# alibaba/TorchEasyRec

Hardware: AMD Instinct MI355X
Metric: samples/sec DLRM-Criteo (examples/dlrm_criteo.config) training, batch 65536 global (higher is better)
Workload: dtype f32; 1 GPU; dlrm_criteo: 26 tables x dim 16 (204.2M rows, fp32), fused sparse adagrad + dense Adam, ids uniform; global_batch=65536, per_rank_batch=65536, parallelism=single GPU, all tables local (table-wise on one rank), row_layout=interleaved

## Files before the change

include/tzrec_hip.h:

```cpp
#ifndef TZREC_HIP_H_
#define TZREC_HIP_H_

#include <stddef.h>
#include <stdint.h>

#ifdef __cplusplus
extern "C" {
#endif

#define TZR_DT_F32 0
#define TZR_DT_F16 1

#define TZR_OK 0
#define TZR_ERR_INVALID (-1)
#define TZR_ERR_LAUNCH (-2)
#define TZR_ERR_WORKSPACE (-3)
#define TZR_ERR_UNSUPPORTED (-4)

#define TZR_MAX_DST 8
#define TZR_MAX_FEAT_DST 4

#define TZR_POOL_SUM 0
#define TZR_POOL_MEAN 1

// ... 556 lines not shown
                            float* d_grad_sparse, int64_t grad_sparse_stride, void* stream);

int tzr_dot_interaction_top_supported(int F, int D, int has_dense, int H);
int tzr_dot_interaction_top_fwd(const float* d_dense, int64_t dense_stride, const float* d_sparse,
                                int64_t sparse_stride, int F, int D, int64_t B, const float* d_W1, int64_t ldw,
                                const float* d_bias, int H, int relu, float* d_z, int64_t z_stride, float* d_y1,
                                int64_t y1_stride, void* stream);
int tzr_dot_interaction_top_bwd(const float* d_dense, int64_t dense_stride, const float* d_sparse,
                                int64_t sparse_stride, int F, int D, int64_t B, const float* d_g1, int64_t g1_stride,
                                int H, const float* d_W1, int64_t ldw, const float* d_scale, float* d_grad_dense,
                                int64_t grad_dense_stride, float* d_grad_sparse, int64_t grad_sparse_stride,
                                void* stream);
int tzr_ia_top_packed_floats(void);
int tzr_ia_top_pack_w1(const float* d_W1, int64_t ldw, int n, float* d_fwd_packed, float* d_bwd_packed, void* stream);
int tzr_dot_interaction_top_fwd_packed(const float* d_dense, int64_t dense_stride, const float* d_sparse,
                                       int64_t sparse_stride, int F, int D, int64_t B, const float* d_W1, int64_t ldw,
                                       const float* d_bias, int H, int relu, float* d_z, int64_t z_stride, float* d_y1,
                                       int64_t y1_stride, const float* d_W1_fwd_packed, void* stream);
int tzr_dot_interaction_top_bwd_packed(const float* d_dense, int64_t dense_stride, const float* d_sparse,
                                       int64_t sparse_stride, int F, int D, int64_t B, const float* d_g1, int64_t g1_stride,
                                       int H, const float* d_W1, int64_t ldw, const float* d_scale, float* d_grad_dense,
                                       int64_t grad_dense_stride, float* d_grad_sparse, int64_t grad_sparse_stride,
                                       const float* d_W1_bwd_packed, void* stream);

int64_t tzr_dot_interaction_top_wgrad_workspace(int F, int D, int has_dense, int H);
int tzr_dot_interaction_top_wgrad(const float* d_dense, int64_t dense_stride, const float* d_sparse,
                                  int64_t sparse_stride, int F, int D, int64_t B, const float* d_g1, int64_t g1_stride,
                                  int H, const float* d_scale, float* d_dW1, int64_t ldw, void* d_ws, int64_t ws_bytes,
                                  void* stream);

int tzr_fm_fwd(const float* d_x, int64_t x_stride, int F, int D, int64_t B, float* d_out,
               int64_t out_stride, void* stream);
int tzr_fm_bwd(const float* d_x, int64_t x_stride, int F, int D, int64_t B,
               const float* d_grad_out, int64_t grad_out_stride, float* d_grad_x,
               int64_t grad_x_stride, void* stream);

#define TZR_METRIC_MAX_THRESHOLDS 4096
int tzr_metric_update(const float* d_probs, const int64_t* d_labels, int64_t B, const float* d_thresholds, int T,
                      uint64_t* d_hist, double* d_ne, void* stream);

int tzr_grouped_auc_append(const float* d_probs, const int64_t* d_labels, const int64_t* d_keys, int64_t B,
                           float* d_row_probs, int32_t* d_row_labels, int64_t* d_row_keys, int64_t capacity,
                           int64_t* d_state, void* stream);

size_t tzr_grouped_auc_reduce_workspace(int64_t n);
int tzr_grouped_auc_reduce(const int64_t* d_keys, const float* d_probs, const int32_t* d_labels, int64_t n,
// ... 7 lines not shown
```

torcheasyrec_amd/_lib.py:

```python
from __future__ import annotations

import ctypes as C
import os
from typing import Optional

import numpy as np
import torch

_HERE = os.path.dirname(os.path.abspath(__file__))
LIB_PATH = os.path.join(_HERE, "libtzrec_hip.so")

TZR_OK = 0
TZR_ERR_INVALID, TZR_ERR_UNSUPPORTED = -1, -4
TZR_MAX_DST = 8
TZR_MAX_FEAT_DST = 4
METRIC_MAX_THRESHOLDS = 4096
POOL_SUM, POOL_MEAN = 0, 1
DT_F32, DT_F16 = 0, 1
FWD_MIXED_DTYPE = 1
OPT_SGD, OPT_ADAGRAD, OPT_ROWWISE_ADAGRAD, OPT_ACCUMULATE, OPT_ADAM = 0, 1, 2, 3, 4
OPT_PARTIAL_ROWWISE_ADAM, OPT_LAMB, OPT_PARTIAL_ROWWISE_LAMB, OPT_LARS_SGD = 5, 6, 7, 8
OPT_ADADELTA, OPT_RMSPROP = 9, 10
ABI_VERSION = 15
WD_NONE, WD_L2, WD_DECOUPLE = 0, 1, 2
# ... 176 lines not shown
    "tzr_dense_adam_fused_w1": (_i32, [C.POINTER(TzrAdamTensor), C.POINTER(TzrAdamSource), _i32, C.POINTER(TzrWgradParts), _vp, C.c_float,
                                       C.c_float, C.c_float, C.c_float, C.c_float, C.POINTER(TzrPackedW1), _vp]),
    "tzr_dense_optim_fused": (_i32, [C.POINTER(TzrDenseOptTensor), C.POINTER(TzrAdamSource), _i32, C.POINTER(TzrDenseOptGroup), _i32,
                                     C.POINTER(TzrWgradParts), _vp]),
    "tzr_mlp2_bwd_parts": (_i32, [_vp, _i64, _vp, _i64, _vp, _i64, _vp, _i64, _i64, _i32, _i32, _i32, _vp, _vp, _sz, C.POINTER(C.c_int),
                                  C.POINTER(C.c_int), _vp]),
    "tzr_dot_interaction_top_wgrad_parts": (_i32, [_vp, _i64, _vp, _i64, _i32, _i32, _i64, _vp, _i64, _i32, _vp, _vp, _i64,
                                                   C.POINTER(TzrWgradParts), _vp]),
    "tzr_dot_interaction_fwd": (_i32, [_vp, _i64, _vp, _i64, _i32, _i32, _i64, _vp, _i64, _i32,
                                       _i32, _vp]),
    "tzr_dot_interaction_bwd": (_i32, [_vp, _i64, _vp, _i64, _i32, _i32, _i64, _vp, _i64, _i32,
                                       _i32, _vp, _i64, _vp, _i64, _vp]),
    "tzr_dot_interaction_top_supported": (_i32, [_i32, _i32, _i32, _i32]),
    "tzr_dot_interaction_top_fwd": (_i32, [_vp, _i64, _vp, _i64, _i32, _i32, _i64, _vp, _i64, _vp, _i32, _i32, _vp, _i64,
                                           _vp, _i64, _vp]),
    "tzr_dot_interaction_top_bwd": (_i32, [_vp, _i64, _vp, _i64, _i32, _i32, _i64, _vp, _i64, _i32, _vp, _i64, _vp, _vp,
                                           _i64, _vp, _i64, _vp]),
    "tzr_ia_top_packed_floats": (_i32, []),
    "tzr_ia_top_pack_w1": (_i32, [_vp, _i64, _i32, _vp, _vp, _vp]),
    "tzr_dot_interaction_top_fwd_packed": (_i32, [_vp, _i64, _vp, _i64, _i32, _i32, _i64, _vp, _i64, _vp, _i32, _i32, _vp, _i64,
                                                  _vp, _i64, _vp, _vp]),
    "tzr_dot_interaction_top_bwd_packed": (_i32, [_vp, _i64, _vp, _i64, _i32, _i32, _i64, _vp, _i64, _i32, _vp, _i64, _vp, _vp,
                                                  _i64, _vp, _i64, _vp, _vp]),
    "tzr_dot_interaction_top_wgrad_workspace": (_i64, [_i32, _i32, _i32, _i32]),
    "tzr_dot_interaction_top_wgrad": (_i32, [_vp, _i64, _vp, _i64, _i32, _i32, _i64, _vp, _i64, _i32, _vp, _vp, _i64, _vp,
                                             _i64, _vp]),
    "tzr_jagged_to_padded_dense": (_i32, [_vp, _i64, _vp, _i64, _i64, _i32, C.c_float, _vp, _vp]),
    "tzr_padded_dense_to_jagged": (_i32, [_vp, _vp, _i64, _i64, _i32, _vp, _i64, _vp]),
    "tzr_quantize_rows_q8f16": (_i32, [_vp, _i32, _i64, _i64, _i32, _vp, _vp, _vp]),
    "tzr_dequantize_rows_q8f16": (_i32, [_vp, _i64, _i32, _vp, _i64, _vp]),
    "tzr_segment_reduce_fwd": (_i32, [_vp, _i64, _vp, _i64, _i32, _i32, _vp, _i64, _vp]),
    "tzr_segment_reduce_bwd": (_i32, [_vp, _i64, _vp, _i64, _i32, _i32, _vp, _i64, _vp]),
    "tzr_jagged_segment_ids": (_i32, [_vp, _i64, _i64, _vp, _vp]),
    "tzr_din_assemble_fwd": (_i32, [_vp, _i64, _vp, _i64, _vp, _i64, _i64, _i32, _vp, _i64, _vp]),
    "tzr_din_assemble_bwd": (_i32, [_vp, _i64, _vp, _i64, _vp, _i64, _vp, _vp, _i64, _i64, _i32, _vp, _i64, _i32, _vp, _i64, _vp]),
    "tzr_din_assemble2_fwd": (_i32, [_vp, _i64, _vp, _i64, _vp, _i64, _i64, _i32, _vp, _i64, _vp]),
    "tzr_din_assemble2_bwd": (_i32, [_vp, _i64, _vp, _i64, _vp, _i64, _vp, _vp, _i64, _i64, _i32, _vp, _i64, _i32, _vp, _i64, _vp, _i64, _vp]),
    "tzr_din_attn_fwd": (_i32, [_vp, _i64, _i32, _vp, _vp, _vp, _i64, _i32, _vp, _i64, _i64, _vp, _i64, _vp, _vp]),
    "tzr_din_attn_bwd": (_i32, [_vp, _i64, _vp, _vp, _i64, _i32, _vp, _i64, _i64, _vp, _vp, _i64, _vp]),
    "tzr_jagged_dot_attn_fwd": (_i32, [_vp, _i64, _vp, _i64, _i32, _vp, _i64, _i64, _i64, _vp, _i64, _vp, _vp]),
    "tzr_jagged_dot_attn_bwd": (_i32, [_vp, _i64, _vp, _vp, _i64, _vp, _i64, _i32, _vp, _i64, _i64, _i64, _vp, _i64, _vp, _i64, _vp]),
    "tzr_jagged_pool_fwd": (_i32, [_vp, _i64, _i32, _vp, _i64, _i64, _i64, _i32, _vp, _i64, _vp]),
    "tzr_jagged_pool_bwd": (_i32, [_vp, _i64, _i32, _vp, _i64, _i64, _i64, _i32, _vp, _i64, _vp]),
    "tzr_cross_fwd": (_i32, [_vp, _i64, _vp, _vp, _i32, _i64, _i32, _vp, _i64, _vp, _vp]),
    "tzr_cross_bwd_workspace": (_sz, [_i64, _i32, _i32]),
    "tzr_cross_bwd": (_i32, [_vp, _i64, _vp, _i64, _vp, _vp, _vp, _i32, _i64, _i32, _vp, _i64, _vp, _vp, _vp, _sz, _vp]),
# ... 228 lines not shown
```

torcheasyrec_amd/csrc/interaction_top.hip:

```cpp
#include "tzr_common.h"
#include "interaction_pack.h"
#include <type_traits>
#include <tzr_gfx950.h>

#define IT_THREADS 1024
#define IT_WAVES (IT_THREADS / TZR_WAVE)
#define IT_TS 16
#define IT_H 64
#define IT_KS (IT_H / 4)
#define IT_D 16
#define IT_MAXBLK 64
#define IT_BPW (IT_MAXBLK / IT_WAVES)
#define IT_KB (IT_MAXBLK / 4)
#define IT_MAX_BATCH (int64_t(1) << 30)
#define IT_N_CRITEO 27
#define IT_SROW 33
#define IT_SS (32 * IT_SROW + 4)
#define IT_PS (32 * IT_D)
#define IT_XS (32 * (IT_D + 1))
#define IT_ZP (16 * IT_MAXBLK + 4)
#define IT_YP (IT_H + 1)

typedef float it_f32x4 __attribute__((ext_vector_type(4)));

// ... 549 lines not shown
      }
      const int64_t b = t * IT_TS + s;
      if (b < a.B) {
        a.y1[b * a.y1_stride + h] = v0;
        a.y1[b * a.y1_stride + h + 1] = v1;
      }
    }
    IT_PROF_MARK(5);
  }
  IT_PROF_DUMP(a.prof);
}

#define IT_C_P (IT_N_CRITEO * (IT_N_CRITEO - 1) / 2)
#define IT_C_NPB ((IT_C_P + 15) / 16)
#define IT_C_NBLK (IT_C_NPB + IT_N_CRITEO)
#define IT_C_ZP (16 * IT_C_NBLK + 4 + TZR_WAVE)
#define IT_C_ZT (IT_TS * IT_C_ZP)
#define IT_C_YT (4 * IT_TS * IT_YP)
static_assert(IT_C_NBLK == 4 * 12 + 1, "twelve whole blocks per K-group and one k-step of the 49th");
static_assert(2 * IT_C_ZT + 2 * IT_C_YT <= 2 * IT_TS * IT_ZP + IT_C_YT, "fits the forward's LDS");
static_assert(IT_C_ZT * 4 < 65536 && IT_C_YT * 4 < 65536, "the other buffer is an immediate offset of a DS instruction");
static_assert(IT_PACK_N == IT_N_CRITEO && IT_PACK_P == IT_C_P && IT_PACK_NPB == IT_C_NPB && IT_PACK_H == IT_H, "interaction_pack.h describes this shape");

__device__ __forceinline__ void it_fwd_criteo(const ItFwdArgs& a, float* __restrict__ Zs, float* __restrict__ Ys, int lane, int wv) {
  constexpr int n = IT_N_CRITEO, P = IT_C_P, npb = IT_C_NPB, NB = 12;
  const int r = lane & 15, q = lane >> 4;
  const int kg = wv >> 2, hb = wv & 3;
  const int vfirst = kg * NB;
  float Wf[NB][4];
  float Wx[1];
  IT_PROF_PRO_BEGIN;
  if (a.W1p) {
#pragma unroll
    for (int m = 0; m < NB; ++m) {
      const float4 w = tzr_ld4(a.W1p + it_pack_fwd_off(wv, m, lane));
      Wf[m][0] = w.x; Wf[m][1] = w.y; Wf[m][2] = w.z; Wf[m][3] = w.w;
    }
    Wx[0] = a.W1p[it_pack_fwd_x_off(wv, lane)];
    IT_PROF_PRO_END(a.prof);
    for (int k = threadIdx.x; k < 2 * IT_TS * IT_C_ZP; k += IT_THREADS) Zs[k] = 0.f;
    __syncthreads();
  } else {
    it_fwd_stage_w<NB, 1, IT_C_ZP>(a, Zs, Wf, Wx, n, P, npb, NB, 1, vfirst, vfirst + NB, r, q, kg, hb IT_PROF_PRO_ARG);
  }
  const int Bn = (int)a.B;
  const int ntiles = (Bn + IT_TS - 1) / IT_TS;
  const int G = gridDim.x;
  int t = blockIdx.x;
  if (t >= ntiles) return;
  float* const zrow = Zs + wv * IT_C_ZP;
  float* tg[12];
  {
    float* const slot = zrow + 16 * IT_C_NBLK + 4 + lane;
#pragma unroll
    for (int reg = 0; reg < 4; ++reg) {
      const int i0 = 4 * q + reg, i1 = 16 + i0, j0 = r, j1 = 16 + r;
      const int b0 = i0 * (2 * n - i0 - 1) / 2 - i0 - 1, b1 = i1 * (2 * n - i1 - 1) / 2 - i1 - 1;
      tg[3 * reg + 0] = (i0 < j0) ? zrow + b0 + j0 : slot;
      tg[3 * reg + 1] = (j1 < n) ? zrow + b0 + j1 : slot;
      tg[3 * reg + 2] = (i1 < j1 && j1 < n) ? zrow + b1 + j1 : slot;
    }
  }
  const int rr1 = 16 + r < n ? 16 + r : n - 1;
  float* const xs0 = zrow + 16 * npb + IT_D * r + 4 * q;
  float* const xs1 = zrow + 16 * npb + IT_D * rr1 + 4 * q;
  const float* const zr = Zs + r * IT_C_ZP + 4 * q + 16 * vfirst;
  const float* const zx = Zs + r * IT_C_ZP + 4 * q + 16 * (4 * NB) + kg;
  float* const yw = Ys + kg * (IT_TS * IT_YP) + (4 * q) * IT_YP + 16 * hb + r;
  const float* const yr = Ys + wv * IT_YP + lane;
  const bool lo_dense = a.hd && r == 0;
  const unsigned lo_off = (unsigned)((r > a.hd ? r - a.hd : 0) * IT_D + 4 * q), hi_off = (unsigned)((rr1 - a.hd) * IT_D + 4 * q);
  auto fetch = [&](int tt) {
    const int bi = tt * IT_TS + wv;
    const int64_t b = bi < Bn ? bi : Bn - 1;
    const float* sp = a.sparse + b * a.sparse_stride;
    ItX x;
    x.lo = tzr_ld4(lo_dense ? a.dense + b * a.dense_stride + 4 * q : sp + lo_off);
    x.hi = tzr_ld4(sp + hi_off);
    return x;
  };
  auto row = [&](const ItX& X, const int zo) {
    it_f32x4 c00 = {0.f, 0.f, 0.f, 0.f}, c01 = c00, c11 = c00;
    const float x0[4] = {X.lo.x, X.lo.y, X.lo.z, X.lo.w};
    const float x1[4] = {X.hi.x, X.hi.y, X.hi.z, X.hi.w};
#pragma unroll
    for (int e = 0; e < 4; ++e) {
      c00 = __builtin_amdgcn_mfma_f32_16x16x4f32(x0[e], x0[e], c00, 0, 0, 0);
      c01 = __builtin_amdgcn_mfma_f32_16x16x4f32(x0[e], x1[e], c01, 0, 0, 0);
      c11 = __builtin_amdgcn_mfma_f32_16x16x4f32(x1[e], x1[e], c11, 0, 0, 0);
    }
#pragma unroll
    for (int reg = 0; reg < 4; ++reg) {
      tg[3 * reg + 0][zo] = c00[reg];
      tg[3 * reg + 1][zo] = c01[reg];
      tg[3 * reg + 2][zo] = c11[reg];
    }
    tzr_st4(xs0 + zo, X.lo);
    tzr_st4(xs1 + zo, X.hi);
  };
  row(fetch(t), 0);
  ItX X = fetch(t + G < ntiles ? t + G : t);
  float bias = a.bias ? a.bias[lane] : 0.f;
  TZR_OPAQUE(bias);
  struct Part { float p[4]; };
  auto sum_load = [&](const int yo) {
    Part s;
#pragma unroll
    for (int g = 0; g < 4; ++g) s.p[g] = yr[yo + g * (IT_TS * IT_YP)];
    return s;
  };
  auto sum_store = [&](int tt, const Part& s) {
    float v = bias;
#pragma unroll
    for (int g = 0; g < 4; ++g) v += s.p[g];
    if (a.relu) v = v > 0.f ? v : 0.f;
    const int b = tt * IT_TS + wv;
    if (b < Bn) a.y1[(int64_t)b * a.y1_stride + lane] = v;
  };
  const bool row_first_wave = a.stagger == 0 ? ((wv >> 2) & 1) != 0 : a.stagger == 1;
  IT_PROF_DECL;
  auto tile = [&](auto CUR, auto RF, bool prev) {
    constexpr int cur = decltype(CUR)::value;
    constexpr bool row_first = decltype(RF)::value;
    constexpr int zo = cur * IT_C_ZT, zn = (cur ^ 1) * IT_C_ZT, yo = cur * IT_C_YT, yp = (cur ^ 1) * IT_C_YT;
    auto product = [&]() {
      it_f32x4 acc = {0.f, 0.f, 0.f, 0.f};
      float4 av[2];
      av[0] = tzr_ld4(zr + zo);
#pragma unroll
      for (int m = 0; m < NB; ++m) {
        if (m + 1 < NB) av[(m + 1) & 1] = tzr_ld4(zr + zo + 16 * (m + 1));
        const float4 c = av[m & 1];
        acc = __builtin_amdgcn_mfma_f32_16x16x4f32(c.x, Wf[m][0], acc, 0, 0, 0);
        acc = __builtin_amdgcn_mfma_f32_16x16x4f32(c.y, Wf[m][1], acc, 0, 0, 0);
        acc = __builtin_amdgcn_mfma_f32_16x16x4f32(c.z, Wf[m][2], acc, 0, 0, 0);
        acc = __builtin_amdgcn_mfma_f32_16x16x4f32(c.w, Wf[m][3], acc, 0, 0, 0);
        __builtin_amdgcn_sched_barrier(0);
      }
      acc = __builtin_amdgcn_mfma_f32_16x16x4f32(zx[zo], Wx[0], acc, 0, 0, 0);
#pragma unroll
      for (int j = 0; j < 4; ++j) yw[yo + j * IT_YP] = acc[j];
    };
    auto next_row = [&]() {
      if (t + G < ntiles) row(X, zn);
      X = fetch(t + 2 * G < ntiles ? t + 2 * G : t);
    };
    tzr_lds_barrier();
    IT_PROF_MARK(0);
    if (row_first) {
      next_row();
      IT_PROF_MARK(1);
      if (prev) sum_store(t - G, sum_load(yp));
      IT_PROF_MARK(5);
      product();
      IT_PROF_MARK(2);
    } else {
      Part s;
      if (prev) s = sum_load(yp);
      __builtin_amdgcn_sched_barrier(0);
      product();
      IT_PROF_MARK(2);
      if (prev) sum_store(t - G, s);
      IT_PROF_MARK(5);
      next_row();
      IT_PROF_MARK(3);
    }
  };
  int last = 0;
// ... 8 lines not shown
      t += G;
      last = 1;
      if (t >= ntiles) break;
      prev = true;
    }
  };
  if (row_first_wave) run(std::true_type());
  else run(std::false_type());
  tzr_lds_barrier();
  sum_store(t - G, sum_load(last * IT_C_YT));
  IT_PROF_DUMP(a.prof);
}

template <bool ZOUT>
__device__ __forceinline__ void it_fwd_body(const ItFwdArgs& a) {
  constexpr int kZCriteo = 2 * IT_TS * (16 * 49 + 4), kYs = 4 * IT_TS * IT_YP;
  __shared__ __attribute__((aligned(16))) float Sm[2 * IT_TS * IT_ZP + kYs];
  __shared__ float trash[IT_THREADS];
  const int lane = threadIdx.x & (TZR_WAVE - 1);
  const int wv = __builtin_amdgcn_readfirstlane((int)(threadIdx.x / TZR_WAVE));
  float* tr = trash + threadIdx.x;
  if (a.n == IT_N_CRITEO) {
    if (ZOUT) it_fwd_loop<12, 1, ZOUT, IT_N_CRITEO>(a, Sm, Sm + kZCriteo, tr, lane, wv);
    else it_fwd_criteo(a, Sm, Sm + 2 * IT_C_ZT, lane, wv);
  } else {
    it_fwd_loop<IT_KB, 3, ZOUT, 0>(a, Sm, Sm + 2 * IT_TS * IT_ZP, tr, lane, wv);
  }
}

__global__ __launch_bounds__(IT_THREADS) void tzr_ia_top_fwd_kernel(ItFwdArgs a) { it_fwd_body<false>(a); }
__global__ __launch_bounds__(IT_THREADS) void tzr_ia_top_fwd_z_kernel(ItFwdArgs a) { it_fwd_body<true>(a); }

int g_tzr_it_fwd_stagger = 0;
int g_tzr_it_wgs = 0;

static unsigned it_grid(int64_t B) {
  const int64_t cus = g_tzr_it_wgs > 0 ? g_tzr_it_wgs : 256;
  const int64_t tiles = (B + IT_TS - 1) / IT_TS;
  return (unsigned)(tiles < cus ? (tiles < 1 ? 1 : tiles) : cus);
}

extern "C" int tzr_dot_interaction_top_supported(int F, int D, int has_dense, int H) {
  const int n = F + (has_dense ? 1 : 0);
  if (D != IT_D || H != IT_H || n < 2 || n > 32) return 0;
  return ((n * (n - 1) / 2 + 15) / 16 + n) <= IT_MAXBLK ? 1 : 0;
}

__global__ __launch_bounds__(256) void tzr_ia_top_pack_w1_kernel(const float* __restrict__ W1, int64_t ldw, float* __restrict__ fwd,
                                                                 float* __restrict__ bwd) {
  const int idx = blockIdx.x * 256 + threadIdx.x;
  if (idx >= IT_PACK_H * IT_PACK_VCOLS) return;
  const int h = idx / IT_PACK_VCOLS, vc = idx - h * IT_PACK_VCOLS;
  const int col = it_real_col(vc, IT_PACK_P, IT_PACK_NPB, IT_PACK_NPB + IT_PACK_N);
  const float w = col >= 0 ? W1[(int64_t)h * ldw + col] : 0.f;
// ... 82 lines not shown
  a.W1p = (n == IT_N_CRITEO && !d_z) ? d_W1_fwd_packed : nullptr;
  a.dense = d_dense; a.sparse = d_sparse; a.W1 = d_W1; a.bias = d_bias; a.z = d_z; a.y1 = d_y1;
  a.dense_stride = dense_stride; a.sparse_stride = sparse_stride; a.ldw = ldw; a.z_stride = z_stride; a.y1_stride = y1_stride;
  a.B = B; a.n = n; a.hd = hd; a.relu = relu;
  a.stagger = g_tzr_it_fwd_stagger > 0 ? g_tzr_it_fwd_stagger - 1 : 0;
#ifdef IT_PROF
  a.prof = g_tzr_it_prof;
#else
  a.prof = nullptr;
#endif
  if (d_z) hipLaunchKernelGGL(tzr_ia_top_fwd_z_kernel, dim3(it_grid(B)), dim3(IT_THREADS), 0, st, a);
  else hipLaunchKernelGGL(tzr_ia_top_fwd_kernel, dim3(it_grid(B)), dim3(IT_THREADS), 0, st, a);
  TZR_CHECK_LAUNCH();
  return TZR_OK;
}

extern "C" int tzr_dot_interaction_top_fwd(const float* d_dense, int64_t dense_stride, const float* d_sparse,
                                           int64_t sparse_stride, int F, int D, int64_t B, const float* d_W1,
                                           int64_t ldw, const float* d_bias, int H, int relu, float* d_z,
                                           int64_t z_stride, float* d_y1, int64_t y1_stride, void* stream) {
  return tzr_dot_interaction_top_fwd_packed(d_dense, dense_stride, d_sparse, sparse_stride, F, D, B, d_W1, ldw, d_bias, H, relu, d_z, z_stride,
                                            d_y1, y1_stride, nullptr, stream);
}
```

torcheasyrec_amd/dense.py:

```python
from __future__ import annotations

import collections
import contextlib
import dataclasses
import os
import weakref
from typing import Iterable, List, Optional, Tuple

import ctypes as C

import torch

from . import _lib


class _BceLogitsFn(torch.autograd.Function):
    @staticmethod
    def forward(ctx, logits, labels, sample_weight):
        x = logits.contiguous().float()
        y = labels.contiguous()
        if y.dtype not in (torch.float32, torch.int32, torch.int64):
            y = y.float()
        loss = torch.empty((), dtype=torch.float32, device=x.device)
        grad = torch.empty_like(x)
# ... 694 lines not shown
    return e


class _InteractionTopLossFn(torch.autograd.Function):

    @staticmethod
    def forward(ctx, dense, sparse, D, W1, b1, W2, b2, w3, b3, labels):
        B = sparse.shape[0]
        F = sparse.shape[1] // D
        sparse = sparse.contiguous()
        dense = dense.contiguous()
        n = F + 1
        width = n * (n - 1) // 2 + D * n
        H1 = W1.shape[0]
        dev = sparse.device
        y1 = torch.empty(B, H1, dtype=torch.float32, device=dev)
        z = None if _owned_wgrad(B, sparse.shape[1]) else torch.empty(B, width, dtype=torch.float32, device=dev)
        W1_, b1_ = _f32c(W1), _f32c(b1)
        pk = _fresh_packed_w1(W1_) if (n == 27 and D == 16 and H1 == 64) else None
        _lib.check(_lib.lib().tzr_dot_interaction_top_fwd_packed(
            _lib.ptr(dense), dense.stride(0), _lib.ptr(sparse), sparse.stride(0), F, D, B, _lib.ptr(W1_), W1_.stride(0),
            _lib.ptr(b1_), H1, 1, _lib.ptr(z), width, _lib.ptr(y1), y1.stride(0), _lib.ptr(pk.fwd) if pk is not None else None,
            _lib.stream_ptr(dev)), "tzr_dot_interaction_top_fwd_packed")
        ctx.w1_packed = pk
        logits, g1, dW2, db2, dw3, scal, db1 = _mlp_tail(y1, labels, W2, b2, w3, b3)
        ctx.save_for_backward(dense, sparse, W1_, g1, dW2, db2, dw3, scal, db1)
        ctx.z = z
        ctx.cfg = (F, D)
        ctx.w1_ref = W1
        ctx.mark_non_differentiable(logits)
        ctx.set_materialize_grads(False)
        return scal[1], logits

    @staticmethod
    def backward(ctx, gl, _glogits):
        dense, sparse, W1, g1, dW2, db2, dw3, scal, db1 = ctx.saved_tensors
        F, D = ctx.cfg
        B = sparse.shape[0]
        root = _loss_is_root(gl)
        gl32 = None if root else gl.reshape(1).to(torch.float32)
        gd = gs = None
        if ctx.needs_input_grad[0] or ctx.needs_input_grad[1]:
            gs = torch.empty_like(sparse)
            gd = torch.empty_like(dense)
            pk = ctx.w1_packed
            _lib.check(_lib.lib().tzr_dot_interaction_top_bwd_packed(
                _lib.ptr(dense), dense.stride(0), _lib.ptr(sparse), sparse.stride(0), F, D, B, _lib.ptr(g1), g1.stride(0),
                g1.shape[1], _lib.ptr(W1), W1.stride(0), _lib.ptr(gl32), _lib.ptr(gd), gd.stride(0), _lib.ptr(gs),
                gs.stride(0), _lib.ptr(pk.bwd) if pk is not None else None, _lib.stream_ptr(sparse.device)),
                "tzr_dot_interaction_top_bwd_packed")
        if not ctx.needs_input_grad[3]:
            dW1 = None
        elif ctx.z is None:
            dW1 = interaction_top_wgrad(dense, sparse, D, g1, gl32, defer_for=(ctx.w1_ref,))
        else:
            dW1 = weight_grad(g1, ctx.z) if root else weight_grad(g1, ctx.z) * gl
        if root:
            return (gd, gs, None, dW1, db1, dW2, db2, dw3, scal[0:1], None)
        outs = torch._foreach_mul([db1, dW2, db2, dw3, scal[0:1]], gl)
        return (gd, gs, None, dW1, *outs, None)


def interaction_top_wgrad(dense: torch.Tensor, sparse: torch.Tensor, D: int, g1: torch.Tensor,
                          scale: Optional[torch.Tensor] = None, defer_for=None) -> torch.Tensor:
    B = sparse.shape[0]
    F = sparse.shape[1] // D
    n = F + 1
    width = n * (n - 1) // 2 + D * n
    H = g1.shape[1]
    if B == 0:
        return torch.zeros(H, width, dtype=torch.float32, device=sparse.device)
    dW = torch.empty(H, width, dtype=torch.float32, device=sparse.device)
    L = _lib.lib()
    ws = _lib.workspace(L.tzr_dot_interaction_top_wgrad_workspace(F, D, 1, H), sparse.device)
    if defer_for is not None and _defer_finish(sparse.device, defer_for):
        blob = _lib.TzrWgradParts()
        _lib.check(L.tzr_dot_interaction_top_wgrad_parts(
            _lib.ptr(dense), dense.stride(0), _lib.ptr(sparse), sparse.stride(0), F, D, B, _lib.ptr(g1), g1.stride(0), H,
            _lib.ptr(scale), _lib.ptr(ws), ws.numel(), C.byref(blob), _lib.stream_ptr(sparse.device)), "tzr_dot_interaction_top_wgrad_parts")
        _defer(dW, "wgrad", (ws, scale), blob, defer_for)
        return dW
    _lib.check(L.tzr_dot_interaction_top_wgrad(
        _lib.ptr(dense), dense.stride(0), _lib.ptr(sparse), sparse.stride(0), F, D, B, _lib.ptr(g1), g1.stride(0), H,
# ... 209 lines not shown
```

torcheasyrec_amd/dlrm.py:

```python
from __future__ import annotations

from typing import Dict, List, Optional, Sequence

import torch
from torch import nn

from .embedding import EmbeddingBagCollection, EmbeddingBagConfig, SparseOptimizerConfig
from .interaction import FactorizationMachine, dot_interaction
from .sparse import KeyedJaggedTensor


import os

_GEMV_OUTPUT = os.environ.get("TZR_OUTPUT_GEMV", "1") == "1"
_FUSED_HEAD_BWD = os.environ.get("TZR_FUSED_HEAD_BWD", "1") == "1"
_FUSED_RELU_BWD = os.environ.get("TZR_MLP_FUSED_RELU_BWD", "1") == "1"
_FUSED_RELU = os.environ.get("TZR_MLP_FUSED_RELU", "1") == "1"
_FUSED_MLP2 = os.environ.get("TZR_FUSED_MLP2", "1") == "1"
_FUSED_TOP_LOSS = os.environ.get("TZR_FUSED_TOP_LOSS", "1") == "1"
_FUSED_IA_TOP = os.environ.get("TZR_FUSED_IA_TOP", "1") == "1"
_FUSED_IA_TOP_MIN_B = int(os.environ.get("TZR_FUSED_IA_TOP_MIN_B", "0"))


def _on_emulator() -> bool:
# ... 213 lines not shown

    def predict_from_embeddings(self, dense: torch.Tensor, sparse: torch.Tensor) -> torch.Tensor:
        d = self.dense_mlp(dense)
        if (not torch.is_grad_enabled() and _FUSED_IA_TOP and self.final_mlp._plain and self.arch_with_sparse
                and (sparse.is_cuda or _on_emulator()) and sparse.shape[0] >= _FUSED_IA_TOP_MIN_B):
            from .dense import interaction_first_layer, interaction_top_fits

            lin = self.final_mlp.linears()
            if interaction_top_fits(d, sparse, self.dim, lin[0]):
                y = interaction_first_layer(d, sparse, self.dim, lin[0])
                for l in lin[1:]:
                    y = torch.relu(l(y))
                return self.output_mlp(y).squeeze(1)
        allf = dot_interaction(d, sparse, self.dim, cat_dense=True, cat_sparse=self.arch_with_sparse)
        return self.output_mlp(self.final_mlp(allf)).squeeze(1)

    def forward(self, dense: torch.Tensor, sparse_features: KeyedJaggedTensor) -> torch.Tensor:
        sparse = self.ebc.forward_grouped(sparse_features)["sparse"]
        return self.predict_from_embeddings(dense, sparse)

    def loss_from_embeddings(self, dense: torch.Tensor, sparse: torch.Tensor, labels: torch.Tensor):
        return head_loss(self, dense, sparse, labels)

    def forward_loss(self, dense: torch.Tensor, sparse_features: KeyedJaggedTensor, labels: torch.Tensor):
        sparse = self.ebc.forward_grouped(sparse_features)["sparse"]
        return self.loss_from_embeddings(dense, sparse, labels)


class DeepFM(nn.Module):

    def __init__(
        self,
        tables: Sequence[EmbeddingBagConfig],
        groups: Dict[str, List[str]],
        dense_dim: int,
        fm_dim: int,
        deep_mlp: Sequence[int] = (512, 256, 128),
        final_mlp: Optional[Sequence[int]] = (64,),
        num_class: int = 1,
        device: Optional[torch.device] = None,
        sparse_optimizer: Optional[SparseOptimizerConfig] = None,
    ) -> None:
        super().__init__()
        self.ebc = EmbeddingBagCollection(tables, device=device, optimizer=sparse_optimizer, groups=groups)
        self.has_fm_group = "fm" in groups
        self.fm_dim = fm_dim
        dims = self.ebc._out_dim
# ... 36 lines not shown
```

torcheasyrec_amd/embedding.py:

```python
from __future__ import annotations

import math
import os
from dataclasses import dataclass, field
from typing import Callable, Dict, List, Optional, Sequence, Tuple

import numpy as np
import torch
from torch import nn

from . import _lib, opt_kinds
from .sparse import KeyedJaggedTensor, KeyedTensor
from .sparse_bwd import SparseBackward, cells_geometry, direct_supported, grad_dsts


@dataclass
class EmbeddingBagConfig:

    name: str
    embedding_dim: int
    num_embeddings: int
    feature_names: List[str] = field(default_factory=list)
    pooling: str = "sum"
    init_fn: Optional[Callable[[torch.Tensor], None]] = None
# ... 138 lines not shown

class _Table(nn.Module):
    def __init__(self, weight: torch.Tensor) -> None:
        super().__init__()
        self.weight = nn.Parameter(weight, requires_grad=False)


@dataclass
class _Lookup:
    key: str
    table: int
    out_key: str


class _Meta:

    def __init__(self) -> None:
        self.tables_np = self.feats_np = self.slots_np = None
        self.d_tables = self.d_feats = self.d_slots = None
        self.d_bwd_tables = self.d_bwd_feats = None
        self.bwd_tables_np = self.bwd_feats_np = None
        self.n_keys = 0
        self.cells: Dict[int, Optional["_CellsGeo"]] = {}


class _CellsGeo:

    def __init__(self, image: np.ndarray, info, device: torch.device) -> None:
        self.h_img = image
        self.h_ptr = image.ctypes.data
        self.n_chunks, self.n_units = int(info[1]), int(info[2])
        self.d_img = _lib.workspace(image.nbytes, device)[:image.nbytes]
        self.d_img.copy_(torch.from_numpy(image))
        off = int(info[6])
        self.d_overflow = self.d_img[off:off + 4].view(torch.int32)
        pin = device.type == "cuda"
        self.h_overflow = torch.zeros(1, dtype=torch.int32, pin_memory=pin)
        self.seen = 0
        self.copied = None
        self.launches = 0
        self.demoted = False


@dataclass(slots=True)
class _Plan:

# ... 12 lines not shown
    dead = [int(i) for i in by_order if not (feats[i]["table"] >= 0 and not frozen[int(feats[i]["table"])])]
    for o, i in enumerate(live + dead):
        bf[i]["order"] = o
    for i in dead:
        bf[i]["table"] = -1
    for t in range(len(bt)):
        mine = [i for i in live if int(feats[i]["table"]) == t]
        bt[t]["first_order"] = int(bf[mine[0]]["order"]) if mine else 0
        bt[t]["n_feats"] = len(mine)
    return bt, bf


class _PooledLookupFn(torch.autograd.Function):
    @staticmethod
    def forward(ctx, ebc, kjt, dst_names, hook):
        outs = ebc._launch_forward(kjt, dst_names, with_plan=True)
        ctx.ebc, ctx.kjt, ctx.dst_names = ebc, kjt, dst_names
        return tuple(outs)

    @staticmethod
    def backward(ctx, *grads):
        ctx.ebc._launch_backward(ctx.kjt, ctx.dst_names, grads)
        return None, None, None, None


class EmbeddingBagCollection(nn.Module):

    def __init__(
        self,
        tables: Sequence[EmbeddingBagConfig],
        device: Optional[torch.device] = None,
        optimizer: Optional[SparseOptimizerConfig] = None,
        groups: Optional[Dict[str, List[str]]] = None,
        row_layout: str = "interleaved",
    ) -> None:
        super().__init__()
        device = torch.device(device) if device is not None else torch.device("cpu")
        self._device = device
        self._configs = list(tables)
        self._opt_cfg = optimizer
        self._row_layout = row_layout
        self.embedding_bags = nn.ModuleDict()
        self._storage: List[torch.Tensor] = []
        self._states: Dict[str, torch.Tensor] = {}
        self._lookups: List[_Lookup] = []
        names = set()
# ... 5 lines not shown
            if cfg.embedding_dim % 4 or cfg.embedding_dim > 256:
                raise ValueError(f"{cfg.name}: embedding_dim must be a multiple of 4, <= 256")
            for f in cfg.feature_names:
                feat_tables.setdefault(f, []).append(t)
        for t, cfg in enumerate(self._configs):
            for f in cfg.feature_names:
                out_key = f if len(feat_tables[f]) == 1 else f"{f}@{cfg.name}"
                self._lookups.append(_Lookup(f, t, out_key))
        self._out_dim = {lk.out_key: self._configs[lk.table].embedding_dim for lk in self._lookups}
        self._allocate()
        self._has_fp16 = any(m.weight.dtype == torch.float16 for m in self.embedding_bags.values())
        self._groups = groups
        self._dst_layouts: Dict[Tuple[str, ...], List[Tuple[str, List[str]]]] = {}
        self._meta_cache: Dict[Tuple, _Meta] = {}
        self.fused_optimizer = FusedSparseOptimizer(optimizer, self) if optimizer is not None else None
        self._hook = torch.zeros(0, requires_grad=True, device=device)
        self._timers = None
        self._side_stream = None
        self._lookup_trackers: list = []
        self._track_segs: Dict[Tuple[str, ...], tuple] = {}
        self.async_plan = False
        self.forward_plan = os.environ.get("TZR_FWD_PLAN", "1") != "0"
        self.forward_plans = 0
        self.expect_hot_rows = False
        self._dims = (max(c.num_embeddings for c in self._configs), max(c.embedding_dim for c in self._configs))
        self._direct_ws: Dict[int, torch.Tensor] = {}
        self.plan_mode = os.environ.get("TZR_BWD_PLAN", "auto")
        if self.plan_mode not in ("auto", "cells", "exact"):
            raise ValueError("TZR_BWD_PLAN: auto | cells | exact")

    CELLS_PROBATION = 4

    def _cells_geometry(self, meta: _Meta, B: int) -> Optional[_CellsGeo]:
        if B in meta.cells:
            return meta.cells[B]
        made = cells_geometry(meta.bwd_tables_np, meta.bwd_feats_np, B, self._bwd_dims()[1])
        geo = None if made is None else _CellsGeo(*made, self._device)
        meta.cells[B] = geo
        return geo

    def reset_plan_mode(self) -> None:
        for meta in self._meta_cache.values():
            for geo in meta.cells.values():
                if geo is not None:
                    if geo.copied is not None:
                        geo.copied.synchronize()
# ... 351 lines not shown
        keys = tuple(kjt.keys())
        segs = self._track_segs.get(keys)
        if segs is None:
            index = {k: i for i, k in enumerate(keys)}
            segs = tuple((self._configs[lk.table].name, index[lk.key]) for lk in self._lookups if lk.key in index)
            self._track_segs[keys] = segs
        uniform, offsets = self._kjt_args(kjt)
        for fn in self._lookup_trackers:
            fn(self, segs, kjt.values(), offsets, kjt.stride(), 1 if uniform else 0)

    def _run(self, kjt: KeyedJaggedTensor, dst_names: Tuple[str, ...]) -> List[torch.Tensor]:
        if kjt.uniform_length() is None and getattr(kjt, "_uniform_keys", None):
            view = kjt.uniform_prefix([lk.key for lk in self._lookups])
            if view is not None:
                kjt = view
        if self._lookup_trackers:
            self._notify_trackers(kjt)
        if torch.is_grad_enabled() and self.fused_optimizer is not None and self.training:
            if self.async_plan and getattr(kjt, "_tzr_plan", None) is None:
                self.plan_backward_async(kjt, dst_names)
            return list(_PooledLookupFn.apply(self, kjt, dst_names, self._hook))
        return self._launch_forward(kjt, dst_names)

    def forward(self, features: KeyedJaggedTensor) -> KeyedTensor:
        (out,) = self._run(features, ("__all__",))
        keys = [lk.out_key for lk in self._lookups]
        return KeyedTensor(keys, [self._out_dim[k] for k in keys], out)

    def forward_grouped(self, features: KeyedJaggedTensor, group_names: Optional[Sequence[str]] = None) -> Dict[str, torch.Tensor]:
        if self._groups is None:
            raise ValueError("EmbeddingBagCollection was built without groups")
        names = tuple(group_names) if group_names is not None else tuple(self._groups)
        outs = self._run(features, names)
        return dict(zip(names, outs))

    def bounds_check(self, features: KeyedJaggedTensor, mode: int = _lib.BOUNDS_WARNING) -> torch.Tensor:
        meta = self._meta(features.keys(), self._default_layout())
        cnt = torch.zeros(1, dtype=torch.int64, device=self._device)
        rc = _lib.lib().tzr_bounds_check(
            _lib.ptr(meta.d_tables), _lib.ptr(meta.d_feats), len(self._lookups),
            _lib.ptr(features.values()), _lib.ptr(features.offsets()), features.stride(), mode,
            _lib.ptr(cnt), _lib.stream_ptr(self._device),
        )
        _lib.check(rc, "tzr_bounds_check")
        return cnt
```

Baseline: 143.6 million samples/s.

## Fuse embedding gather into interaction-top forward kernel for DLRM Criteo

Adds a gather variant of the Criteo interaction-top forward kernel. It reads ids, looks up embedding rows straight from the tables, computes the interaction and first linear layer, and writes the pooled sparse output for backward. This removes the separate embedding-bag forward kernel and the extra round trip of the pooled activations through memory. A deferred autograd lookup hooks the embedding backward onto the gradient. The path is narrow (26 features, dim 16, one id per bag, fp32) and adds register and latency pressure to the fused kernel, with an id-prefetch pipeline.

Result: faster. 149.7 million samples/s, median of 6 (+4.2%).

```diff
diff --git a/include/tzrec_hip.h b/include/tzrec_hip.h
--- a/include/tzrec_hip.h
+++ b/include/tzrec_hip.h
@@ -602,6 +602,10 @@
                                        int H, const float* d_W1, int64_t ldw, const float* d_scale, float* d_grad_dense,
                                        int64_t grad_dense_stride, float* d_grad_sparse, int64_t grad_sparse_stride,
                                        const float* d_W1_bwd_packed, void* stream);
+int tzr_dot_interaction_top_fwd_gather(const TzrTable* d_tables, const TzrFeature* d_feats, int n_feats, const int64_t* d_values,
+                                       int64_t n_values, int D, int64_t B, const float* d_dense, int64_t dense_stride,
+                                       const float* d_W1_fwd_packed, const float* d_bias, int H, int relu, float* d_sparse_out,
+                                       int64_t sparse_stride, float* d_y1, int64_t y1_stride, void* stream);
 
 int64_t tzr_dot_interaction_top_wgrad_workspace(int F, int D, int has_dense, int H);
 int tzr_dot_interaction_top_wgrad(const float* d_dense, int64_t dense_stride, const float* d_sparse,
diff --git a/torcheasyrec_amd/_lib.py b/torcheasyrec_amd/_lib.py
--- a/torcheasyrec_amd/_lib.py
+++ b/torcheasyrec_amd/_lib.py
@@ -222,6 +222,8 @@
                                                   _vp, _i64, _vp, _vp]),
     "tzr_dot_interaction_top_bwd_packed": (_i32, [_vp, _i64, _vp, _i64, _i32, _i32, _i64, _vp, _i64, _i32, _vp, _i64, _vp, _vp,
                                                   _i64, _vp, _i64, _vp, _vp]),
+    "tzr_dot_interaction_top_fwd_gather": (_i32, [_vp, _vp, _i32, _vp, _i64, _i32, _i64, _vp, _i64, _vp, _vp, _i32, _i32, _vp, _i64,
+                                                  _vp, _i64, _vp]),
     "tzr_dot_interaction_top_wgrad_workspace": (_i64, [_i32, _i32, _i32, _i32]),
     "tzr_dot_interaction_top_wgrad": (_i32, [_vp, _i64, _vp, _i64, _i32, _i32, _i64, _vp, _i64, _i32, _vp, _vp, _i64, _vp,
                                              _i64, _vp]),
diff --git a/torcheasyrec_amd/csrc/interaction_top.hip b/torcheasyrec_amd/csrc/interaction_top.hip
--- a/torcheasyrec_amd/csrc/interaction_top.hip
+++ b/torcheasyrec_amd/csrc/interaction_top.hip
@@ -595,7 +595,24 @@
 static_assert(IT_C_ZT * 4 < 65536 && IT_C_YT * 4 < 65536, "the other buffer is an immediate offset of a DS instruction");
 static_assert(IT_PACK_N == IT_N_CRITEO && IT_PACK_P == IT_C_P && IT_PACK_NPB == IT_C_NPB && IT_PACK_H == IT_H, "interaction_pack.h describes this shape");
 
-__device__ __forceinline__ void it_fwd_criteo(const ItFwdArgs& a, float* __restrict__ Zs, float* __restrict__ Ys, int lane, int wv) {
+struct ItGather {
+  const TzrTable* tables;
+  const TzrFeature* feats;
+  const int64_t* values;
+  float* out;
+  int64_t out_stride;
+};
+struct ItIds {
+  uint2 lo, hi;
+};
+struct ItSrc {
+  const char* base;
+  uint32_t rows, rstride, key8, pad;
+};
+
+template <bool GATHER>
+__device__ __forceinline__ void it_fwd_criteo(const ItFwdArgs& a, const ItGather& ga, ItSrc* __restrict__ srcs, float* __restrict__ Zs,
+                                              float* __restrict__ Ys, int lane, int wv) {
   constexpr int n = IT_N_CRITEO, P = IT_C_P, npb = IT_C_NPB, NB = 12;
   const int r = lane & 15, q = lane >> 4;
   const int kg = wv >> 2, hb = wv & 3;
@@ -603,7 +620,7 @@
   float Wf[NB][4];
   float Wx[1];
   IT_PROF_PRO_BEGIN;
-  if (a.W1p) {
+  if (GATHER || a.W1p) {
 #pragma unroll
     for (int m = 0; m < NB; ++m) {
       const float4 w = tzr_ld4(a.W1p + it_pack_fwd_off(wv, m, lane));
@@ -611,6 +628,23 @@
     }
     Wx[0] = a.W1p[it_pack_fwd_x_off(wv, lane)];
     IT_PROF_PRO_END(a.prof);
+    if constexpr (GATHER) {
+      const int i = threadIdx.x;
+      if (i < n) {
+        int f = 0;
+#pragma unroll
+        for (int k = 0; k < n - 1; ++k) f = ga.feats[k].col[0] == IT_D * (i > 0 ? i - 1 : 0) ? k : f;
+        const TzrFeature ft = ga.feats[f];
+        const TzrTable tb = ga.tables[ft.table];
+        ItSrc sr;
+        sr.base = i > 0 ? reinterpret_cast<const char*>(tb.w) : reinterpret_cast<const char*>(a.dense);
+        sr.rows = tb.rows > 0x7fffffff ? 0x7fffffffu : (uint32_t)tb.rows;
+        sr.rstride = (i > 0 ? (uint32_t)tb.w_stride : (uint32_t)a.dense_stride) * 4u;
+        sr.key8 = (uint32_t)ft.key * (uint32_t)a.B * 8u;
+        sr.pad = 0;
+        srcs[i] = sr;
+      }
+    }
     for (int k = threadIdx.x; k < 2 * IT_TS * IT_C_ZP; k += IT_THREADS) Zs[k] = 0.f;
     __syncthreads();
   } else {
@@ -652,6 +686,39 @@
     x.hi = tzr_ld4(sp + hi_off);
     return x;
   };
+  const char *lo_base = nullptr, *hi_base = nullptr;
+  uint32_t lo_rows = 0, hi_rows = 0, lo_rstride = 0, hi_rstride = 0, lo_key8 = 0, hi_key8 = 0;
+  if constexpr (GATHER) {
+    const ItSrc sl = srcs[r], sh = srcs[rr1];
+    lo_base = sl.base + 16 * q; lo_rows = sl.rows; lo_rstride = sl.rstride; lo_key8 = sl.key8;
+    hi_base = sh.base + 16 * q; hi_rows = sh.rows; hi_rstride = sh.rstride; hi_key8 = sh.key8;
+  }
+  const bool lo_is_dense = r == 0;
+  auto sample = [&](int tt) {
+    const int bi = tt * IT_TS + wv;
+    return (uint32_t)(bi < Bn ? bi : Bn - 1);
+  };
+  auto fetch_ids = [&](int tt) {
+    const char* vb = reinterpret_cast<const char*>(ga.values + sample(tt));
+    ItIds I;
+    I.lo = tzr_ldg8(vb + lo_key8);
+    I.hi = tzr_ldg8(vb + hi_key8);
+    return I;
+  };
+  auto fetch_rows = [&](const ItIds& I, int tt) {
+    uint32_t il = (I.lo.y == 0u && I.lo.x < lo_rows) ? I.lo.x : 0u;
+    const uint32_t ih = (I.hi.y == 0u && I.hi.x < hi_rows) ? I.hi.x : 0u;
+    il = lo_is_dense ? sample(tt) : il;
+    ItX x;
+    x.lo = tzr_ldg4(reinterpret_cast<const float*>(lo_base + (uint64_t)il * lo_rstride));
+    x.hi = tzr_ldg4(reinterpret_cast<const float*>(hi_base + (uint64_t)ih * hi_rstride));
+    return x;
+  };
+  auto store_rows = [&](const ItX& x, int tt) {
+    float* so = ga.out + (int64_t)sample(tt) * ga.out_stride;
+    if (!lo_is_dense) tzr_stg4(so + lo_off, x.lo);
+    tzr_stg4(so + hi_off, x.hi);
+  };
   auto row = [&](const ItX& X, const int zo) {
     it_f32x4 c00 = {0.f, 0.f, 0.f, 0.f}, c01 = c00, c11 = c00;
     const float x0[4] = {X.lo.x, X.lo.y, X.lo.z, X.lo.w};
@@ -671,8 +738,20 @@
     tzr_st4(xs0 + zo, X.lo);
     tzr_st4(xs1 + zo, X.hi);
   };
-  row(fetch(t), 0);
-  ItX X = fetch(t + G < ntiles ? t + G : t);
+  ItX X;
+  ItIds I;
+  if constexpr (GATHER) {
+    const int t1 = t + G < ntiles ? t + G : t;
+    const ItIds I0 = fetch_ids(t), I1 = fetch_ids(t1);
+    I = fetch_ids(t + 2 * G < ntiles ? t + 2 * G : t);
+    const ItX X0 = fetch_rows(I0, t);
+    X = fetch_rows(I1, t1);
+    row(X0, 0);
+    store_rows(X0, t);
+  } else {
+    row(fetch(t), 0);
+    X = fetch(t + G < ntiles ? t + G : t);
+  }
   float bias = a.bias ? a.bias[lane] : 0.f;
   TZR_OPAQUE(bias);
   struct Part { float p[4]; };
@@ -715,8 +794,19 @@
       for (int j = 0; j < 4; ++j) yw[yo + j * IT_YP] = acc[j];
     };
     auto next_row = [&]() {
-      if (t + G < ntiles) row(X, zn);
-      X = fetch(t + 2 * G < ntiles ? t + 2 * G : t);
+      if constexpr (GATHER) {
+        TZR_OPAQUE(I.lo.x); TZR_OPAQUE(I.lo.y); TZR_OPAQUE(I.hi.x); TZR_OPAQUE(I.hi.y);
+        if (t + G < ntiles) {
+          row(X, zn);
+          store_rows(X, t + G);
+        }
+        const int t2 = t + 2 * G < ntiles ? t + 2 * G : t;
+        X = fetch_rows(I, t2);
+        I = fetch_ids(t + 3 * G < ntiles ? t + 3 * G : t2);
+      } else {
+        if (t + G < ntiles) row(X, zn);
+        X = fetch(t + 2 * G < ntiles ? t + 2 * G : t);
+      }
     };
     tzr_lds_barrier();
     IT_PROF_MARK(0);
@@ -771,7 +861,7 @@
   float* tr = trash + threadIdx.x;
   if (a.n == IT_N_CRITEO) {
     if (ZOUT) it_fwd_loop<12, 1, ZOUT, IT_N_CRITEO>(a, Sm, Sm + kZCriteo, tr, lane, wv);
-    else it_fwd_criteo(a, Sm, Sm + 2 * IT_C_ZT, lane, wv);
+    else it_fwd_criteo<false>(a, ItGather{}, nullptr, Sm, Sm + 2 * IT_C_ZT, lane, wv);
   } else {
     it_fwd_loop<IT_KB, 3, ZOUT, 0>(a, Sm, Sm + 2 * IT_TS * IT_ZP, tr, lane, wv);
   }
@@ -779,6 +869,13 @@
 
 __global__ __launch_bounds__(IT_THREADS) void tzr_ia_top_fwd_kernel(ItFwdArgs a) { it_fwd_body<false>(a); }
 __global__ __launch_bounds__(IT_THREADS) void tzr_ia_top_fwd_z_kernel(ItFwdArgs a) { it_fwd_body<true>(a); }
+__global__ __launch_bounds__(IT_THREADS) void tzr_ia_top_fwd_gather_kernel(ItFwdArgs a, ItGather ga) {
+  __shared__ __attribute__((aligned(16))) float Sm[2 * IT_C_ZT + 2 * IT_C_YT];
+  const int lane = threadIdx.x & (TZR_WAVE - 1);
+  const int wv = __builtin_amdgcn_readfirstlane((int)(threadIdx.x / TZR_WAVE));
+  __shared__ ItSrc srcs[IT_N_CRITEO];
+  it_fwd_criteo<true>(a, ga, srcs, Sm, Sm + 2 * IT_C_ZT, lane, wv);
+}
 
 int g_tzr_it_fwd_stagger = 0;
 int g_tzr_it_wgs = 0;
@@ -907,3 +1004,33 @@
   return tzr_dot_interaction_top_fwd_packed(d_dense, dense_stride, d_sparse, sparse_stride, F, D, B, d_W1, ldw, d_bias, H, relu, d_z, z_stride,
                                             d_y1, y1_stride, nullptr, stream);
 }
+
+extern "C" int tzr_dot_interaction_top_fwd_gather(const TzrTable* d_tables, const TzrFeature* d_feats, int n_feats, const int64_t* d_values,
+                                                  int64_t n_values, int D, int64_t B, const float* d_dense, int64_t dense_stride,
+                                                  const float* d_W1_fwd_packed, const float* d_bias, int H, int relu, float* d_sparse_out,
+                                                  int64_t sparse_stride, float* d_y1, int64_t y1_stride, void* stream) {
+  if (!d_tables || !d_feats || !d_values || !d_dense || !d_W1_fwd_packed || !d_sparse_out || !d_y1 || n_feats <= 0 || B < 0) return TZR_ERR_INVALID;
+  if (n_feats != IT_N_CRITEO - 1 || D != IT_D || H != IT_H) return TZR_ERR_UNSUPPORTED;
+  if (sparse_stride < (int64_t)n_feats * IT_D || n_values < (int64_t)n_feats * B) return TZR_ERR_INVALID;
+  if ((sparse_stride & 3) || (dense_stride & 3) ||
+      ((reinterpret_cast<uintptr_t>(d_sparse_out) | reinterpret_cast<uintptr_t>(d_dense) | reinterpret_cast<uintptr_t>(d_W1_fwd_packed)) & 15) ||
+      (reinterpret_cast<uintptr_t>(d_values) & 7) || (reinterpret_cast<uintptr_t>(d_y1) & 3))
+    return TZR_ERR_INVALID;
+  if (B > IT_MAX_BATCH || B * sparse_stride >= (int64_t(1) << 30) || n_values >= (int64_t(1) << 29)) return TZR_ERR_UNSUPPORTED;
+  if (B == 0) return TZR_OK;
+  ItFwdArgs a;
+  a.dense = d_dense; a.sparse = nullptr; a.W1 = nullptr; a.bias = d_bias; a.W1p = d_W1_fwd_packed; a.z = nullptr; a.y1 = d_y1;
+  a.dense_stride = dense_stride; a.sparse_stride = 0; a.ldw = 0; a.z_stride = 0; a.y1_stride = y1_stride;
+  a.B = B; a.n = IT_N_CRITEO; a.hd = 1; a.relu = relu;
+  a.stagger = g_tzr_it_fwd_stagger > 0 ? g_tzr_it_fwd_stagger - 1 : 0;
+#ifdef IT_PROF
+  a.prof = g_tzr_it_prof;
+#else
+  a.prof = nullptr;
+#endif
+  ItGather ga;
+  ga.tables = d_tables; ga.feats = d_feats; ga.values = d_values; ga.out = d_sparse_out; ga.out_stride = sparse_stride;
+  hipLaunchKernelGGL(tzr_ia_top_fwd_gather_kernel, dim3(it_grid(B)), dim3(IT_THREADS), 0, static_cast<hipStream_t>(stream), a, ga);
+  TZR_CHECK_LAUNCH();
+  return TZR_OK;
+}
diff --git a/torcheasyrec_amd/dense.py b/torcheasyrec_amd/dense.py
--- a/torcheasyrec_amd/dense.py
+++ b/torcheasyrec_amd/dense.py
@@ -740,6 +740,10 @@
             _lib.ptr(dense), dense.stride(0), _lib.ptr(sparse), sparse.stride(0), F, D, B, _lib.ptr(W1_), W1_.stride(0),
             _lib.ptr(b1_), H1, 1, _lib.ptr(z), width, _lib.ptr(y1), y1.stride(0), _lib.ptr(pk.fwd) if pk is not None else None,
             _lib.stream_ptr(dev)), "tzr_dot_interaction_top_fwd_packed")
+        return _InteractionTopLossFn._finish(ctx, dense, sparse, F, D, W1, W1_, pk, z, y1, W2, b2, w3, b3, labels)
+
+    @staticmethod
+    def _finish(ctx, dense, sparse, F, D, W1, W1_, pk, z, y1, W2, b2, w3, b3, labels):
         ctx.w1_packed = pk
         logits, g1, dW2, db2, dw3, scal, db1 = _mlp_tail(y1, labels, W2, b2, w3, b3)
         ctx.save_for_backward(dense, sparse, W1_, g1, dW2, db2, dw3, scal, db1)
@@ -752,13 +756,17 @@
 
     @staticmethod
     def backward(ctx, gl, _glogits):
+        return _InteractionTopLossFn._backward(ctx, gl, ctx.needs_input_grad[0] or ctx.needs_input_grad[1], ctx.needs_input_grad[3])
+
+    @staticmethod
+    def _backward(ctx, gl, need_x, need_w1):
         dense, sparse, W1, g1, dW2, db2, dw3, scal, db1 = ctx.saved_tensors
         F, D = ctx.cfg
         B = sparse.shape[0]
         root = _loss_is_root(gl)
         gl32 = None if root else gl.reshape(1).to(torch.float32)
         gd = gs = None
-        if ctx.needs_input_grad[0] or ctx.needs_input_grad[1]:
+        if need_x:
             gs = torch.empty_like(sparse)
             gd = torch.empty_like(dense)
             pk = ctx.w1_packed
@@ -767,7 +775,7 @@
                 g1.shape[1], _lib.ptr(W1), W1.stride(0), _lib.ptr(gl32), _lib.ptr(gd), gd.stride(0), _lib.ptr(gs),
                 gs.stride(0), _lib.ptr(pk.bwd) if pk is not None else None, _lib.stream_ptr(sparse.device)),
                 "tzr_dot_interaction_top_bwd_packed")
-        if not ctx.needs_input_grad[3]:
+        if not need_w1:
             dW1 = None
         elif ctx.z is None:
             dW1 = interaction_top_wgrad(dense, sparse, D, g1, gl32, defer_for=(ctx.w1_ref,))
@@ -777,6 +785,44 @@
             return (gd, gs, None, dW1, db1, dW2, db2, dw3, scal[0:1], None)
         outs = torch._foreach_mul([db1, dW2, db2, dw3, scal[0:1]], gl)
         return (gd, gs, None, dW1, *outs, None)
+
+
+class _InteractionTopGatherLossFn(torch.autograd.Function):
+
+    @staticmethod
+    def forward(ctx, dense, token, lookup, D, W1, b1, W2, b2, w3, b3, labels):
+        B, F = lookup.B, lookup.n_feats
+        dense = dense.contiguous()
+        dev = dense.device
+        H1 = W1.shape[0]
+        y1 = torch.empty(B, H1, dtype=torch.float32, device=dev)
+        sparse = torch.empty(B, lookup.width, dtype=torch.float32, device=dev)
+        W1_, b1_ = _f32c(W1), _f32c(b1)
+        pk = _fresh_packed_w1(W1_)
+        if pk is None:
+            raise RuntimeError("interaction_top_gather_loss: W1 has no packed copies (interaction_top_gather_fits)")
+        _lib.check(_lib.lib().tzr_dot_interaction_top_fwd_gather(
+            _lib.ptr(lookup.d_tables), _lib.ptr(lookup.d_feats), F, _lib.ptr(lookup.values), lookup.values.numel(), D, B,
+            _lib.ptr(dense), dense.stride(0), _lib.ptr(pk.fwd), _lib.ptr(b1_), H1, 1, _lib.ptr(sparse), sparse.stride(0),
+            _lib.ptr(y1), y1.stride(0), _lib.stream_ptr(dev)), "tzr_dot_interaction_top_fwd_gather")
+        return _InteractionTopLossFn._finish(ctx, dense, sparse, F, D, W1, W1_, pk, None, y1, W2, b2, w3, b3, labels)
+
+    @staticmethod
+    def backward(ctx, gl, _glogits):
+        out = _InteractionTopLossFn._backward(ctx, gl, ctx.needs_input_grad[0] or ctx.needs_input_grad[1], ctx.needs_input_grad[4])
+        return out[:2] + (None,) + out[2:]
+
+
+def interaction_top_gather_fits(n_feats: int, B: int, dense_dim: int, D: int, first_linear) -> bool:
+    W1 = first_linear.weight
+    if n_feats != 26 or D != 16 or dense_dim != D or tuple(W1.shape) != W1_PACKED_SHAPE or W1.dtype != torch.float32:
+        return False
+    return _packed_entry(W1) is not None and _owned_wgrad(B, n_feats * D)
+
+
+def interaction_top_gather_loss(dense, token, lookup, D, l1, l2, out_linear, labels):
+    return _InteractionTopGatherLossFn.apply(dense, token, lookup, D, l1.weight, l1.bias, l2.weight, l2.bias, out_linear.weight,
+                                             out_linear.bias, labels)
 
 
 def interaction_top_wgrad(dense: torch.Tensor, sparse: torch.Tensor, D: int, g1: torch.Tensor,
diff --git a/torcheasyrec_amd/dlrm.py b/torcheasyrec_amd/dlrm.py
--- a/torcheasyrec_amd/dlrm.py
+++ b/torcheasyrec_amd/dlrm.py
@@ -259,7 +259,26 @@
     def loss_from_embeddings(self, dense: torch.Tensor, sparse: torch.Tensor, labels: torch.Tensor):
         return head_loss(self, dense, sparse, labels)
 
+    def _gathering_head(self, dense: torch.Tensor, B: int) -> bool:
+        if not (_FUSED_TOP_LOSS and _FUSED_IA_TOP and self.final_mlp._plain and self.arch_with_sparse and B >= _FUSED_IA_TOP_MIN_B):
+            return False
+        if not (dense.is_cuda or _on_emulator()) or dense.dim() != 2 or dense.dtype != torch.float32 or self.num_sparse != 26:
+            return False
+        from .dense import top_loss_fits
+
+        return top_loss_fits(dense, self.final_mlp.linears(), self.output_mlp)
+
     def forward_loss(self, dense: torch.Tensor, sparse_features: KeyedJaggedTensor, labels: torch.Tensor):
+        if self.ebc.forward_gather and self._gathering_head(dense, sparse_features.stride()):
+            from .dense import interaction_top_gather_fits, interaction_top_gather_loss
+
+            lin = self.final_mlp.linears()
+            if interaction_top_gather_fits(self.num_sparse, sparse_features.stride(), self.dense_mlp.output_dim(), self.dim, lin[0]):
+                deferred = self.ebc.forward_deferred(sparse_features, "sparse")
+                if deferred is not None:
+                    lookup, token = deferred
+                    d = self.dense_mlp(dense)
+                    return interaction_top_gather_loss(d, token, lookup, self.dim, lin[0], lin[1], self.output_mlp, labels)
         sparse = self.ebc.forward_grouped(sparse_features)["sparse"]
         return self.loss_from_embeddings(dense, sparse, labels)
 
diff --git a/torcheasyrec_amd/embedding.py b/torcheasyrec_amd/embedding.py
--- a/torcheasyrec_amd/embedding.py
+++ b/torcheasyrec_amd/embedding.py
@@ -184,6 +184,7 @@
         self.bwd_tables_np = self.bwd_feats_np = None
         self.n_keys = 0
         self.cells: Dict[int, Optional["_CellsGeo"]] = {}
+        self.gather_shape: Optional[bool] = None
 
 
 class _CellsGeo:
@@ -242,6 +243,24 @@
     def backward(ctx, *grads):
         ctx.ebc._launch_backward(ctx.kjt, ctx.dst_names, grads)
         return None, None, None, None
+
+
+class _DeferredLookupFn(torch.autograd.Function):
+
+    @staticmethod
+    def forward(ctx, ebc, kjt, dst_names, hook, B, width):
+        ctx.ebc, ctx.kjt, ctx.dst_names = ebc, kjt, dst_names
+        return hook.new_empty(1).expand(B, width)
+
+    @staticmethod
+    def backward(ctx, grad):
+        ctx.ebc._launch_backward(ctx.kjt, ctx.dst_names, (grad,))
+        return None, None, None, None, None, None
+
+
+class GatherLookup:
+
+    __slots__ = ("d_tables", "d_feats", "n_feats", "values", "B", "width")
 
 
 class EmbeddingBagCollection(nn.Module):
@@ -293,6 +312,8 @@
         self.async_plan = False
         self.forward_plan = os.environ.get("TZR_FWD_PLAN", "1") != "0"
         self.forward_plans = 0
+        self.forward_gather = os.environ.get("TZR_FWD_GATHER", "1") != "0"
+        self.forward_gathers = 0
         self.expect_hot_rows = False
         self._dims = (max(c.num_embeddings for c in self._configs), max(c.embedding_dim for c in self._configs))
         self._direct_ws: Dict[int, torch.Tensor] = {}
@@ -690,6 +711,56 @@
             return list(_PooledLookupFn.apply(self, kjt, dst_names, self._hook))
         return self._launch_forward(kjt, dst_names)
 
+    @staticmethod
+    def _gather_shape(meta: _Meta) -> bool:
+        if meta.gather_shape is None:
+            f, t = meta.feats_np, meta.tables_np
+            meta.gather_shape = bool(
+                len(f) == 26 and (f["n_dst"] == 1).all() and (f["dst"][:, 0] == 0).all()
+                and sorted(int(c) for c in f["col"][:, 0]) == list(range(0, 416, 16))
+                and (t["dim"] == 16).all() and (t["w_dtype"] == _lib.DT_F32).all() and (t["rows"] < (1 << 31)).all() and (t["rows"] > 0).all()
+                and (t["w"] % 16 == 0).all() and (t["w_stride"] % 4 == 0).all())
+        return meta.gather_shape
+
+    def forward_deferred(self, features: KeyedJaggedTensor, group: str) -> Optional[Tuple[GatherLookup, torch.Tensor]]:
+        if not self.forward_gather or self._groups is None or self._has_fp16 or self._timers is not None or self.async_plan:
+            return None
+        if not (torch.is_grad_enabled() and self.fused_optimizer is not None and self.training):
+            return None
+        if self._device.type != "cuda" and _lib.backend() != "emu":
+            return None
+        kjt = features
+        if kjt.uniform_length() is None and getattr(kjt, "_uniform_keys", None):
+            view = kjt.uniform_prefix([lk.key for lk in self._lookups])
+            if view is not None:
+                kjt = view
+        if kjt.uniform_length() != 1 or kjt.weights_or_none() is not None:
+            return None
+        dst_names = (group,)
+        meta = self._meta(kjt.keys(), self._layout_for(dst_names))
+        B, values = kjt.stride(), kjt.values()
+        if not self._gather_shape(meta) or B < 1 or B * 416 >= (1 << 30) or values.numel() >= (1 << 29) or values.dtype != torch.int64:
+            return None
+        p = self._problem(kjt, meta)
+        left = getattr(kjt, "_tzr_plan", None)
+        if left is not None and left.origin == "forward" and left.owner == id(self):
+            kjt._tzr_plan = left = None
+        direct = p.direct_supported()
+        if not direct and self._cells_for(kjt, meta) is None:
+            return None
+        plans = self.forward_plan and not direct and (left is None or left.origin != "caller")
+        if self._lookup_trackers:
+            self._notify_trackers(kjt)
+        if plans:
+            ws, geo = self._plan(kjt, meta, p)
+            kjt._tzr_plan = _Plan(id(self), dst_names, ws, None, geo, "forward")
+            self.forward_plans += 1
+        self.forward_gathers += 1
+        lookup = GatherLookup()
+        lookup.d_tables, lookup.d_feats, lookup.n_feats = meta.d_tables, meta.d_feats, len(meta.feats_np)
+        lookup.values, lookup.B, lookup.width = values, B, 416
+        return lookup, _DeferredLookupFn.apply(self, kjt, dst_names, self._hook, B, 416)
+
     def forward(self, features: KeyedJaggedTensor) -> KeyedTensor:
         (out,) = self._run(features, ("__all__",))
         keys = [lk.out_key for lk in self._lookups]
```
